# rpng/online_lang_splatting

Hardware: AMD Instinct MI355X
Metric: rasterizer fwd+bwd frames/sec @500k Gaussians, 1200x680, 15-dim lang (higher is better)
Workload: dtype f32

## Files before the change

include/olsr.h:

```cpp
#ifndef OLSR_H_INCLUDED
#define OLSR_H_INCLUDED

#include <stddef.h>
#include <stdint.h>

#ifdef __cplusplus
extern "C" {
#endif

#define OLSR_OK 0
#define OLSR_ERR_ARG (-1)
#define OLSR_ERR_DEVICE (-2)
#define OLSR_ERR_ALLOC (-3)
#define OLSR_ERR_CAPACITY (-4)

#define OLSR_STATUS_OK 0
#define OLSR_STATUS_OVERFLOW 1
#define OLSR_STATUS_SYNC_ERROR 2

#define OLSR_BWD_REFERENCE 0
#define OLSR_BWD_EXACT 1

typedef void *(*olsr_alloc_fn)(void *user, size_t nbytes);

// ... 277 lines not shown
  float obs_weight;
  float min_opacity;
  int32_t H, W;
  int32_t feat_layout;
  int32_t _pad0;
  const float *depth, *feat, *opacity;
} olsr_tsdf_view;
int olsr_tsdf_init(const olsr_tsdf_volume *volume, void *hip_stream);
int olsr_tsdf_integrate(const olsr_tsdf_volume *volume, int32_t n_views, const olsr_tsdf_view *views, void *hip_stream);
size_t olsr_tsdf_surface_scratch_bytes(int32_t X, int32_t Y, int32_t Z);
int olsr_tsdf_surface_plan(const olsr_tsdf_volume *volume, float min_weight, void *scratch, int32_t *status,
                           void *hip_stream);
int olsr_tsdf_surface_emit(const olsr_tsdf_volume *volume, float min_weight, const void *scratch, int32_t capacity,
                           float *points, float *feats, int32_t *voxel_index, void *hip_stream);

typedef struct olsr_pose_params {
  double lr_rot, lr_trans, lr_exposure;
  double beta1, beta2, eps;
  double converged_threshold;
  int32_t step;
  int32_t _pad0;
} olsr_pose_params;
int olsr_pose_step(const olsr_pose_params *params, const float *dL_dtau_sum, const float *dL_dexposure,
                   const float *projection_matrix, float *state, int32_t *status, void *hip_stream);
int olsr_pose_step_gated(const olsr_pose_params *params, const float *dL_dtau_sum, const float *dL_dexposure,
                         const float *projection_matrix, float *state, int32_t *status, const int32_t *frame_status,
                         void *hip_stream);

int olsr_accumulate_gradients(int32_t P, int32_t M, int32_t F, int32_t assign,
                              const float *dL_dmeans3D,
                              const float *dL_dsh, const float *dL_dopacity,
                              const float *dL_dscales, const float *dL_drotations,
                              const float *dL_dlanguage, const float *dL_dmeans2D,
                              const int32_t *radii, float *flat, float *densify,
                              int32_t *max_radii, void *hip_stream);

int olsr_sparse_exchange_mask(int32_t P, int32_t width, const float *flat, const uint64_t *row_mask,
                              const int32_t *max_radii, int32_t *imax, void *hip_stream);
int64_t olsr_sparse_exchange_scratch_ints(int32_t P);
int olsr_sparse_exchange_pack(int32_t P, int32_t width, int32_t capacity, const float *flat, const int32_t *imax,
                              int32_t *max_radii, uint64_t *row_mask, const float *densify, int32_t *idx,
                              float *fsum, int32_t *scratch, int32_t *status_dev, void *hip_stream);
int olsr_sparse_exchange_unpack(int32_t P, int32_t width, int32_t capacity, const int32_t *idx, const float *fsum,
                                float *flat, float *densify, void *hip_stream);

int olsr_mark_visible(int32_t P, const float *means3D, const float *viewmatrix,
                      const float *projmatrix, uint8_t *present, void *hip_stream);

const void *olsr_geometry_field(const void *geometry_buffer, int32_t P, int32_t F, const char *name);
const void *olsr_binning_field(const void *binning_buffer, int64_t num_rendered, int32_t F,
                               const char *name);
const void *olsr_image_field(const void *image_buffer, int32_t width, int32_t height, int32_t tile,
                             const char *name);

void olsr_set_profiling(int enable);
int olsr_get_stage_times(const char **names, float *ms, int max);

void olsr_debug_sort_timing(unsigned long long *device_buffer, int max_blocks, int max_launches);

int olsr_debug_sort_plan(int64_t n, int n_is_capacity, int32_t *keys_per_thread, int32_t *blocks);

void olsr_debug_sync_fault(int fault_bits, int spin_limit);

float olsr_debug_rows_ratio(int32_t packed_survivor_waves, float ratio, int32_t *redone_out);

void olsr_debug_sort_knobs(int keys_per_thread, int resident_blocks, int legacy);

void olsr_debug_sort_small(int enable);

void olsr_debug_sort_compact(int enable);

void olsr_debug_composite_stamps(unsigned long long *device_buffer, int capacity);

size_t olsr_debug_backward_ordered_scratch_bytes(int64_t num_rendered, int32_t F);
int olsr_debug_backward_ordered(const olsr_scene *scene, const void *geometry_buffer, int32_t num_rendered,
                                const void *binning_buffer, const void *image_buffer,
                                const float *dL_dout_color, const float *dL_dout_language, const float *dL_dout_depth,
                                void *scratch,
                                float *dL_dmeans2D, float *dL_dconic, float *dL_dopacity, float *dL_dcolors,
                                float *dL_dlanguage, float *dL_ddepths, int32_t condition, void *hip_stream);

int olsr_debug_sort_threads(int threads);

const char *olsr_last_error(void);
const char *olsr_version(void);

#ifdef __cplusplus
}
#endif
#endif
```

online_lang_splatting_amd/_abi.py:

```python
import ctypes as C

OLSR_OK = 0
OLSR_ERR_ARG = -1
OLSR_ERR_DEVICE = -2
OLSR_ERR_ALLOC = -3
OLSR_ERR_CAPACITY = -4

BWD_REFERENCE = 0
BWD_EXACT = 1

ACT_OPACITY_SIGMOID = 1
ACT_SCALE_EXP = 2
ACT_ROTATION_NORMALIZE = 4
ACT_ALL = 7
FLAG_SIGNED_EMPTY_RADII = 1
FLAG_FWD_ACCUM_WEIGHT = 4
FLAG_FRAMES_IN_FLIGHT = 8
FLAG_FWD_ACCUM_MFMA = 2

BINNING_RECT = 0
BINNING_ELLIPSE = 1

SUPPORTED_F = (0, 3, 15, 16, 32)
SUPPORTED_TILES = (15, 16)

ALLOC_FN = C.CFUNCTYPE(C.c_void_p, C.c_void_p, C.c_size_t)

_fp = C.c_void_p


class OlsrScene(C.Structure):

    _fields_ = [
        ("P", C.c_int32),
        ("D", C.c_int32),
        ("M", C.c_int32),
        ("F", C.c_int32),
        ("width", C.c_int32),
        ("height", C.c_int32),
        ("tile", C.c_int32),
        ("prefiltered", C.c_int32),
        ("debug", C.c_int32),
        ("bwd_mode", C.c_int32),
        ("tan_fovx", C.c_float),
        ("tan_fovy", C.c_float),
        ("scale_modifier", C.c_float),
        ("binning", C.c_int32),
        ("background", _fp),
        ("means3D", _fp),
        ("shs", _fp),
        ("colors_precomp", _fp),
        ("language_precomp", _fp),
        ("opacities", _fp),
        ("scales", _fp),
        ("rotations", _fp),
        ("cov3D_precomp", _fp),
        ("viewmatrix", _fp),
        ("projmatrix", _fp),
        ("projmatrix_raw", _fp),
        ("cam_pos", _fp),
        ("activations", C.c_int32),
        ("flags", C.c_int32),
        ("tile_depth_cut", _fp),
        ("backward_row_capacity", C.c_int64),
        ("depth_order_carry", _fp),
    ]


class OlsrGradBucket(C.Structure):

    _fields_ = [("flat", _fp), ("densify", _fp), ("max_radii", _fp), ("assign", C.c_int32), ("_pad0", C.c_int32),
                ("row_mask", _fp)]


class OlsrAdamParams(C.Structure):

    _fields_ = [(n, C.c_double) for n in ("lr_xyz", "lr_sh_dc", "lr_sh_rest", "lr_opacity", "lr_scale", "lr_rotation",
                                           "lr_language", "beta1", "beta2", "eps")] + [("step", C.c_int32), ("_pad0", C.c_int32)]


class OlsrAdamGroupParams(C.Structure):

    _fields_ = [("base", OlsrAdamParams), ("group_step", C.c_int32 * 7), ("skip_mask", C.c_int32)]


ADAM_GROUPS = ("xyz", "f_dc", "f_rest", "opacity", "scaling", "rotation", "f_language")

MAP_EDIT_DENSIFY, MAP_EDIT_MASK = 0, 1


class OlsrMapBuffers(C.Structure):

    _fields_ = [(n, _fp) for n in ("means3D", "shs", "opacities", "scales", "rotations", "language", "exp_avg", "exp_avg_sq",
                                   "kf_id", "n_obs", "stats", "max_radii")]


class OlsrMapEditParams(C.Structure):

    _fields_ = [("mode", C.c_int32), ("n_append", C.c_int32), ("append_kf_id", C.c_int32), ("screen_size_term", C.c_int32),
                ("max_grad", C.c_float), ("min_opacity", C.c_float), ("clone_max_scale", C.c_float), ("big_scale", C.c_float)]


class OlsrPoseParams(C.Structure):

# ... 100 lines not shown
```

online_lang_splatting_amd/_lib.py:

```python
import ctypes as C
import os

from . import _abi

_HERE = os.path.dirname(os.path.abspath(__file__))
LIB_PATH = os.environ.get("OLSR_LIB") or os.path.join(_HERE, "libolsr.so")

EXPORTS = (
    "olsr_geometry_bytes", "olsr_image_bytes", "olsr_binning_bytes", "olsr_backward_scratch_bytes", "olsr_last_forward_token", "olsr_live_rows", "olsr_forward", "olsr_forward_async", "olsr_forward_async_loss", "olsr_fused_loss_scratch_bytes",
    "olsr_backward", "olsr_accumulate_gradients", "olsr_sparse_exchange_mask", "olsr_sparse_exchange_scratch_ints", "olsr_sparse_exchange_pack", "olsr_sparse_exchange_unpack", "olsr_mapping_loss", "olsr_mapping_loss_scratch_bytes", "olsr_tracking_loss", "olsr_refinement_loss", "olsr_refinement_loss_scratch_bytes", "olsr_lang_ae_scratch_bytes", "olsr_lang_ae_train_step", "olsr_lang_ae_encode", "olsr_lang_ae_decode", "olsr_lang_query_scratch_bytes", "olsr_lang_query_sims", "olsr_lang_query_relevancy", "olsr_tsdf_init", "olsr_tsdf_integrate", "olsr_tsdf_surface_scratch_bytes", "olsr_tsdf_surface_plan", "olsr_tsdf_surface_emit", "olsr_pose_step", "olsr_pose_step_gated", "olsr_knn_mean_dist2", "olsr_knn_scratch_bytes", "olsr_adam_step", "olsr_adam_step_sum", "olsr_adam_step_masked", "olsr_adam_step_groups", "olsr_map_edit_scratch_bytes", "olsr_map_edit_plan", "olsr_map_edit_apply", "olsr_bucket_add", "olsr_mark_visible", "olsr_geometry_field", "olsr_binning_field", "olsr_image_field",
    "olsr_set_profiling", "olsr_get_stage_times", "olsr_debug_sort_timing", "olsr_debug_sort_plan", "olsr_debug_sort_knobs", "olsr_debug_sort_small", "olsr_debug_sort_compact", "olsr_debug_sort_threads", "olsr_debug_composite_stamps", "olsr_debug_sync_fault", "olsr_debug_rows_ratio", "olsr_debug_backward_ordered", "olsr_debug_backward_ordered_scratch_bytes", "olsr_live_rows_wait", "olsr_live_rows_overwritten", "olsr_backward_rows", "olsr_last_error", "olsr_version",
)

_lib = None


class OlsrError(RuntimeError):
    def __init__(self, code, msg):
        super().__init__(f"olsr error {code}: {msg}")
        self.code = code


def lib():
    global _lib
    if _lib is not None:
        return _lib
    if not os.path.exists(LIB_PATH):
        raise ImportError(
            f"{LIB_PATH} is missing: build it with `python -m online_lang_splatting_amd.build` "
            "(hipcc, gfx950).  There is no CPU or PyTorch fallback for the rasterizer.")
    L = C.CDLL(LIB_PATH)
    missing = [s for s in EXPORTS if not hasattr(L, s)]
    if missing:
        raise ImportError(f"{LIB_PATH} lacks symbols {missing}; rebuild it")
    vp, i32, i64, sz = C.c_void_p, C.c_int32, C.c_int64, C.c_size_t
    scene_p = C.POINTER(_abi.OlsrScene)
    L.olsr_geometry_bytes.argtypes, L.olsr_geometry_bytes.restype = [i32, i32], sz
    L.olsr_image_bytes.argtypes, L.olsr_image_bytes.restype = [i32, i32, i32], sz
    L.olsr_binning_bytes.argtypes, L.olsr_binning_bytes.restype = [i64, i32], sz
    L.olsr_forward.argtypes = [scene_p, _abi.ALLOC_FN, vp, _abi.ALLOC_FN, vp, _abi.ALLOC_FN, vp,
                               vp, vp, vp, vp, vp, vp, C.POINTER(i32), vp]
    L.olsr_forward.restype = C.c_int
    L.olsr_forward_async.argtypes = [scene_p, vp, vp, i64, vp, vp, vp, vp, vp, vp, vp, vp, vp, vp]
    L.olsr_forward_async.restype = C.c_int
    L.olsr_forward_async_loss.argtypes = [scene_p, vp, vp, i64, vp, vp, vp, vp, vp, vp, vp, vp, vp,
                                          C.POINTER(_abi.OlsrLossFusion), vp]
    L.olsr_forward_async_loss.restype = C.c_int
    L.olsr_fused_loss_scratch_bytes.argtypes, L.olsr_fused_loss_scratch_bytes.restype = [i32, i32, i32], sz
    L.olsr_backward_scratch_bytes.argtypes, L.olsr_backward_scratch_bytes.restype = [i64, i32], sz
    L.olsr_last_forward_token.argtypes, L.olsr_last_forward_token.restype = [], i32
    L.olsr_live_rows.argtypes, L.olsr_live_rows.restype = [i32, i32], i64
    L.olsr_live_rows_wait.argtypes, L.olsr_live_rows_wait.restype = [i32, i32, i32], i64
    L.olsr_live_rows_overwritten.argtypes, L.olsr_live_rows_overwritten.restype = [i32], i32
    L.olsr_backward_rows.argtypes, L.olsr_backward_rows.restype = [i32, i32, i64, i32], i64
    L.olsr_backward.argtypes = ([scene_p, vp, vp, i32, vp, vp, _abi.ALLOC_FN, vp, i32, vp, i64] + [vp] * 3 + [vp] * 13
                                + [C.POINTER(_abi.OlsrGradBucket), vp, vp])
    L.olsr_backward.restype = C.c_int
    L.olsr_accumulate_gradients.argtypes = [i32, i32, i32, i32] + [vp] * 12
    L.olsr_accumulate_gradients.restype = C.c_int
    L.olsr_sparse_exchange_mask.argtypes, L.olsr_sparse_exchange_mask.restype = [i32, i32] + [vp] * 5, C.c_int
    L.olsr_sparse_exchange_scratch_ints.argtypes, L.olsr_sparse_exchange_scratch_ints.restype = [i32], i64
    L.olsr_sparse_exchange_pack.argtypes, L.olsr_sparse_exchange_pack.restype = [i32, i32, i32] + [vp] * 10, C.c_int
    L.olsr_sparse_exchange_unpack.argtypes, L.olsr_sparse_exchange_unpack.restype = [i32, i32, i32] + [vp] * 5, C.c_int
    L.olsr_mapping_loss_scratch_bytes.argtypes, L.olsr_mapping_loss_scratch_bytes.restype = [i32, i32], sz
    L.olsr_mapping_loss.argtypes = [C.POINTER(_abi.OlsrLossParams)] + [vp] * 14
    L.olsr_mapping_loss.restype = C.c_int
    L.olsr_tracking_loss.argtypes = [C.POINTER(_abi.OlsrLossParams)] + [vp] * 13
    L.olsr_tracking_loss.restype = C.c_int
    L.olsr_refinement_loss_scratch_bytes.argtypes, L.olsr_refinement_loss_scratch_bytes.restype = [i32, i32], sz
    L.olsr_refinement_loss.argtypes, L.olsr_refinement_loss.restype = [i32, i32, C.c_float] + [vp] * 6, C.c_int
    L.olsr_lang_ae_scratch_bytes.argtypes, L.olsr_lang_ae_scratch_bytes.restype = [i32], sz
    L.olsr_lang_ae_train_step.argtypes = [C.POINTER(_abi.OlsrLangAeParams), i32] + [vp] * 10
    L.olsr_lang_ae_train_step.restype = C.c_int
    L.olsr_lang_ae_encode.argtypes, L.olsr_lang_ae_encode.restype = [i32, vp, vp, i32, vp, vp], C.c_int
    L.olsr_lang_ae_decode.argtypes, L.olsr_lang_ae_decode.restype = [i32, vp, vp, i32, vp, vp], C.c_int
    qp = C.POINTER(_abi.OlsrLangQueryParams)
    L.olsr_lang_query_scratch_bytes.argtypes, L.olsr_lang_query_scratch_bytes.restype = [qp], sz
    L.olsr_lang_query_sims.argtypes, L.olsr_lang_query_sims.restype = [qp] + [vp] * 6, C.c_int
    L.olsr_lang_query_relevancy.argtypes, L.olsr_lang_query_relevancy.restype = [qp] + [vp] * 11, C.c_int
    tv = C.POINTER(_abi.OlsrTsdfVolume)
    L.olsr_tsdf_init.argtypes, L.olsr_tsdf_init.restype = [tv, vp], C.c_int
    L.olsr_tsdf_integrate.argtypes, L.olsr_tsdf_integrate.restype = [tv, i32, C.POINTER(_abi.OlsrTsdfView), vp], C.c_int
    L.olsr_tsdf_surface_scratch_bytes.argtypes, L.olsr_tsdf_surface_scratch_bytes.restype = [i32, i32, i32], sz
    L.olsr_tsdf_surface_plan.argtypes, L.olsr_tsdf_surface_plan.restype = [tv, C.c_float, vp, vp, vp], C.c_int
    L.olsr_tsdf_surface_emit.argtypes, L.olsr_tsdf_surface_emit.restype = [tv, C.c_float, vp, i32, vp, vp, vp, vp], C.c_int
    L.olsr_pose_step.argtypes = [C.POINTER(_abi.OlsrPoseParams)] + [vp] * 6
    L.olsr_pose_step.restype = C.c_int
    L.olsr_pose_step_gated.argtypes = [C.POINTER(_abi.OlsrPoseParams)] + [vp] * 7
    L.olsr_pose_step_gated.restype = C.c_int
    L.olsr_adam_step.argtypes = [i32, i32, i32, C.POINTER(_abi.OlsrAdamParams)] + [vp] * 10
    L.olsr_adam_step.restype = C.c_int
    L.olsr_adam_step_sum.argtypes = [i32, i32, i32, C.POINTER(_abi.OlsrAdamParams), i32, C.POINTER(vp)] + [vp] * 9
    L.olsr_adam_step_sum.restype = C.c_int
    L.olsr_adam_step_masked.argtypes = [i32, i32, i32, C.POINTER(_abi.OlsrAdamParams), i32, C.POINTER(vp), C.POINTER(vp)] + [vp] * 9
    L.olsr_adam_step_masked.restype = C.c_int
    L.olsr_adam_step_groups.argtypes = [i32, i32, i32, C.POINTER(_abi.OlsrAdamGroupParams), i32, C.POINTER(vp), C.POINTER(vp)] + [vp] * 9
    L.olsr_adam_step_groups.restype = C.c_int
    L.olsr_map_edit_scratch_bytes.argtypes, L.olsr_map_edit_scratch_bytes.restype = [i32], sz
    mb, mp = C.POINTER(_abi.OlsrMapBuffers), C.POINTER(_abi.OlsrMapEditParams)
    L.olsr_map_edit_plan.argtypes, L.olsr_map_edit_plan.restype = [i32, mp, mb, vp, vp, vp, vp], C.c_int
    L.olsr_map_edit_apply.argtypes = [i32, i32, i32, mp, mb, vp, mb, vp, vp, i32, i32, mb, vp, vp]
    L.olsr_map_edit_apply.restype = C.c_int
    L.olsr_bucket_add.argtypes, L.olsr_bucket_add.restype = [i32, i32] + [vp] * 9, C.c_int
    L.olsr_knn_scratch_bytes.argtypes, L.olsr_knn_scratch_bytes.restype = [i32], sz
    L.olsr_knn_mean_dist2.argtypes, L.olsr_knn_mean_dist2.restype = [i32, vp, vp, vp, vp], C.c_int
    L.olsr_mark_visible.argtypes, L.olsr_mark_visible.restype = [i32, vp, vp, vp, vp, vp], C.c_int
    L.olsr_geometry_field.argtypes, L.olsr_geometry_field.restype = [vp, i32, i32, C.c_char_p], vp
    L.olsr_binning_field.argtypes, L.olsr_binning_field.restype = [vp, i64, i32, C.c_char_p], vp
    L.olsr_image_field.argtypes, L.olsr_image_field.restype = [vp, i32, i32, i32, C.c_char_p], vp
    L.olsr_set_profiling.argtypes, L.olsr_set_profiling.restype = [C.c_int], None
    L.olsr_get_stage_times.argtypes = [C.POINTER(C.c_char_p), C.POINTER(C.c_float), C.c_int]
    L.olsr_get_stage_times.restype = C.c_int
    L.olsr_debug_sort_plan.argtypes = [i64, C.c_int, C.POINTER(i32), C.POINTER(i32)]
    L.olsr_debug_sort_plan.restype = C.c_int
    L.olsr_debug_sort_knobs.argtypes = [C.c_int, C.c_int, C.c_int]
    L.olsr_debug_sort_knobs.restype = None
    L.olsr_debug_sort_small.argtypes, L.olsr_debug_sort_small.restype = [C.c_int], None
    L.olsr_debug_sort_compact.argtypes, L.olsr_debug_sort_compact.restype = [C.c_int], None
    L.olsr_debug_sort_threads.argtypes, L.olsr_debug_sort_threads.restype = [C.c_int], C.c_int
    L.olsr_debug_composite_stamps.argtypes, L.olsr_debug_composite_stamps.restype = [vp, C.c_int], None
    L.olsr_debug_sync_fault.argtypes = [C.c_int, C.c_int]
    L.olsr_debug_sync_fault.restype = None
    L.olsr_debug_rows_ratio.argtypes, L.olsr_debug_rows_ratio.restype = [i32, C.c_float, C.POINTER(i32)], C.c_float
    L.olsr_debug_backward_ordered_scratch_bytes.argtypes, L.olsr_debug_backward_ordered_scratch_bytes.restype = [i64, i32], sz
    L.olsr_debug_backward_ordered.argtypes = [scene_p, vp, i32, vp, vp] + [vp] * 3 + [vp] + [vp] * 6 + [i32, vp]
    L.olsr_debug_backward_ordered.restype = C.c_int
    L.olsr_last_error.argtypes, L.olsr_last_error.restype = [], C.c_char_p
    L.olsr_version.argtypes, L.olsr_version.restype = [], C.c_char_p
    _lib = L
    return L


def check(rc):
    if rc != 0:
        raise OlsrError(rc, lib().olsr_last_error().decode())


def stage_times(max_entries=1 << 16):
    names = (C.c_char_p * max_entries)()
    ms = (C.c_float * max_entries)()
    n = lib().olsr_get_stage_times(names, ms, max_entries)
    return [(names[i].decode(), float(ms[i])) for i in range(n)]


def set_profiling(enable):
    lib().olsr_set_profiling(1 if enable else 0)
```

online_lang_splatting_amd/csrc/k_order_carry.hip:

```cpp
#include <cstdlib>

#include "olsr_device.h"
#include "olsr_kernels.h"

namespace olsr {

constexpr int OC_W = 2048;
static_assert(OC_W == 2 * EMIT_CHUNK, "phase B leaves one instance total per emission block");

__device__ __forceinline__ int oc_count_less_front(const u64* __restrict__ B, int n, u64 x) {
  if (!(B[0] < x)) return 0;
  int lo = 0, step = 1;
  while (lo + step < n && B[lo + step] < x) {
    lo += step;
    step <<= 1;
  }
  int hi = lo + step < n ? lo + step : n;
  while (hi - lo > 1) {
    const int mid = (lo + hi) >> 1;
    if (B[mid] < x) lo = mid;
    else hi = mid;
  }
  return hi;
}
__device__ __forceinline__ int oc_count_leq_back(const u64* __restrict__ A, int n, u64 x) {
  if (A[n - 1] <= x) return n;
  int hi = n - 1, step = 1;
  while (hi - step >= 0 && A[hi - step] > x) {
    hi -= step;
    step <<= 1;
  }
  int lo = hi - step >= 0 ? hi - step : -1;
  while (hi - lo > 1) {
    const int mid = (lo + hi) >> 1;
    if (A[mid] <= x) lo = mid;
    else hi = mid;
  }
  return hi;
}

template <int T>
__device__ __forceinline__ u64* oc_window_sort(u64* a, u64* b) {
  constexpr int E = OC_W / T;
  const int tid = threadIdx.x;
#pragma unroll 1
  for (int run = 1; run < OC_W; run <<= 1) {
    u64 x[E];
    int dest[E];
#pragma unroll
    for (int k = 0; k < E; ++k) x[k] = a[tid + k * T];
#pragma unroll
    for (int k = 0; k < E; ++k) {
      const int i = tid + k * T;
      const int base = i & ~(2 * run - 1);
      if ((i & run) == 0) dest[k] = i + oc_count_less_front(a + base + run, run, x[k]);
      else dest[k] = i - run + oc_count_leq_back(a + base, run, x[k]);
    }
#pragma unroll
    for (int k = 0; k < E; ++k) b[dest[k]] = x[k];
    __syncthreads();
    u64* t = a;
    a = b;
    b = t;
  }
  return a;
}

__device__ __forceinline__ u64 oc_pad_low(int l) { return (u64)(u32)l; }
__device__ __forceinline__ u64 oc_pad_high(int l) { return 0xFFFFFFFF00000000ull | (u64)(u32)l; }

template <int T>
__global__ __launch_bounds__(T) void order_repair_a_kernel(int P, const u32* __restrict__ carry,
                                                           const u32* __restrict__ keys, u32* __restrict__ out_key,
                                                           u32* __restrict__ out_gid, u32* __restrict__ miss) {
  constexpr int E = OC_W / T;
  __shared__ __attribute__((aligned(16))) u64 s0[OC_W];
  __shared__ __attribute__((aligned(16))) u64 s1[OC_W];
  const int tid = threadIdx.x;
  const int base = (int)blockIdx.x * OC_W;
  bool bad = false;
#pragma unroll
  for (int k = 0; k < E; ++k) {
    const int l = tid + k * T, i = base + l;
    u64 c = oc_pad_high(l);
    if (i < P) {
      const u32 g = carry[i];
      const bool ok = g < (u32)P;
      bad |= !ok;
      c = ((u64)(ok ? keys[g] : 0xFFFFFFFFu) << 32) | (u64)g;
    }
    s0[l] = c;
  }
  __syncthreads();
  const u64* r = oc_window_sort<T>(s0, s1);
#pragma unroll
  for (int k = 0; k < E; ++k) {
    const int l = tid + k * T, i = base + l;
    if (i < P) {
      const u64 c = r[l];
      out_key[i] = (u32)(c >> 32);
      out_gid[i] = (u32)c;
    }
  }
  if (wave_any(bad) && lane_id() == 0) atomicOr(miss, 1u);
}

template <int T>
__global__ __launch_bounds__(T) void order_repair_b_kernel(int P, const u32* __restrict__ in_key,
                                                           const u32* __restrict__ in_gid, u32* __restrict__ carry,
                                                           const u32* __restrict__ inst_count, u64* __restrict__ totals,
                                                           u32* __restrict__ miss) {
  constexpr int E = OC_W / T;
  __shared__ __attribute__((aligned(16))) u64 s0[OC_W];
  __shared__ __attribute__((aligned(16))) u64 s1[OC_W];
  __shared__ u64 s_tot[2][T / 64];
  const int tid = threadIdx.x, lane = tid & 63, w = tid >> 6;
  const int start = (int)blockIdx.x * OC_W - OC_W / 2;
#pragma unroll
  for (int k = 0; k < E; ++k) {
    const int l = tid + k * T, i = start + l;
    u64 c;
    if (i < 0) c = oc_pad_low(l);
    else if (i < P) c = ((u64)in_key[i] << 32) | (u64)in_gid[i];
    else c = oc_pad_high(l);
    s0[l] = c;
  }
  __syncthreads();
  const u64* r = oc_window_sort<T>(s0, s1);
  bool bad = false;
// ... 68 lines not shown
```

online_lang_splatting_amd/csrc/olsr_device.h:

```cpp
#pragma once
#include <hip/hip_runtime.h>
#include <stdint.h>

#include "olsr_state.h"

namespace olsr {

__host__ __device__ __forceinline__ int32_t rows_stamp_of(long long row_capacity) {
  return row_capacity > 0 ? (int32_t)((row_capacity & 0x3FFFFFFFll) + 1) : 0;
}
__device__ __forceinline__ bool frame_unusable(const int32_t* counters, int32_t rows_stamp = 0) {
  return (counters[CNT_ROW_OVERFLOW] | counters[CNT_SYNC_ERROR]) != 0 ||
         (rows_stamp != 0 && counters[CNT_ROWS_STAMP] != rows_stamp);
}


typedef unsigned int u32;
typedef unsigned long long u64;

__device__ __forceinline__ int lane_id() { return (int)__builtin_amdgcn_mbcnt_hi(~0u, __builtin_amdgcn_mbcnt_lo(~0u, 0u)); }
__device__ __forceinline__ u64 ballot(bool p) { return __builtin_amdgcn_ballot_w64(p); }
__device__ __forceinline__ bool wave_any(bool p) { return ballot(p) != 0ull; }
__device__ __forceinline__ bool wave_all(bool p) { return ballot(!p) == 0ull; }

// ... 46 lines not shown
  float t = swap16_add(swap32_add(a, b), swap32_add(c, d));
  t += dpp_mov<0x128>(t);
  t += dpp_mov<0x124>(t);
  t += dpp_mov<0x122>(t);
  t += dpp_mov<0x121>(t);
  return t;
}
__device__ __forceinline__ float wave_reduce2(float a, float b) {
  float t = swap32_add(a, b);
  t += dpp_mov<0x128>(t);
  t += dpp_mov<0x124>(t);
  t += dpp_mov<0x122>(t);
  t += dpp_mov<0x121>(t);
  t += __builtin_bit_cast(float, __builtin_amdgcn_update_dpp(0, __builtin_bit_cast(int, t), 0x142, 0xa, 0xf, false));
  return t;
}
__device__ __forceinline__ void wave_lds_fence() {
  __builtin_amdgcn_fence(__ATOMIC_RELEASE, "wavefront");
  __builtin_amdgcn_wave_barrier();
}
__device__ __forceinline__ float wave_fold4_lds(float a, float b, float c, float d, float* wl) {
  const int l = lane_id();
  reinterpret_cast<float4*>(wl)[l] = make_float4(a, b, c, d);
  wave_lds_fence();
  const int r = l >> 4, col = l & 15;
  const float* p = wl + 4 * col + (((r & 1) << 1) | (r >> 1));
  const float t = (p[0] + p[64]) + (p[128] + p[192]);
  wave_lds_fence();
  return t;
}
__device__ __forceinline__ float wave_fold2_lds(float a, float b, float* wl) {
  const int l = lane_id();
  reinterpret_cast<float2*>(wl)[l] = make_float2(a, b);
  wave_lds_fence();
  const int r = l >> 4, col = l & 15;
  const float* p = wl + 2 * col + (r >> 1);
  const float t = (p[0] + p[32]) + (p[64] + p[96]);
  wave_lds_fence();
  return t;
}
template <int CTRL>
__device__ __forceinline__ float dpp_quad(float v) {
  return __builtin_bit_cast(float, __builtin_amdgcn_update_dpp(0, __builtin_bit_cast(int, v), CTRL, 0xf, 0xf, true));
}
__device__ __forceinline__ float row_sums3(float t0, float t1, float t2, bool in_hi8, bool in_0to3) {
  const float u0 = t0 + dpp_mov<0x128>(t0);
  const float u1 = t1 + dpp_mov<0x128>(t1);
  const float u2 = t2 + dpp_mov<0x128>(t2);
  float m = in_hi8 ? u1 : u0;
  m += dpp_mov<0x124>(m);
  const float v2 = u2 + dpp_mov<0x124>(u2);
  m = in_0to3 ? v2 : m;
  m += dpp_quad<0x4E>(m);
  m += dpp_quad<0xB1>(m);
  return m;
}
__device__ __forceinline__ float wave_reduce4_lds(float a, float b, float c, float d, float* wl) {
  float t = wave_fold4_lds(a, b, c, d, wl);
  t += dpp_mov<0x128>(t);
  t += dpp_mov<0x124>(t);
  t += dpp_mov<0x122>(t);
  t += dpp_mov<0x121>(t);
  return t;
}
__device__ __forceinline__ float wave_reduce2_lds(float a, float b, float* wl) {
  float t = wave_fold2_lds(a, b, wl);
  t += dpp_mov<0x128>(t);
  t += dpp_mov<0x124>(t);
  t += dpp_mov<0x122>(t);
  t += dpp_mov<0x121>(t);
  return t;
}
typedef float v2f __attribute__((ext_vector_type(2)));
__device__ __forceinline__ int reduce4_lane(int i) { return 16 * (((i & 1) << 1) | ((i >> 1) & 1)); }
__device__ __forceinline__ float lane_read(float v, int lane) {
  return __builtin_bit_cast(float, __builtin_amdgcn_readlane(__builtin_bit_cast(int, v), lane));
}

__device__ __forceinline__ float max_m87(float x) {
  float r;
  asm("v_max_f32 %0, 0xc2ae0000, %1" : "=v"(r) : "v"(x));
  return r;
}
__device__ __forceinline__ float pinned_expf(float x) {
  x = max_m87(x);
  float n = __builtin_rintf(x * 1.44269504088896341f);
  float r = __builtin_fmaf(n, -0.693359375f, x);
  r = __builtin_fmaf(n, 2.12194440e-4f, r);
  float p = 1.9875691500e-4f;
  p = __builtin_fmaf(p, r, 1.3981999507e-3f);
  p = __builtin_fmaf(p, r, 8.3334519073e-3f);
  p = __builtin_fmaf(p, r, 4.1665795894e-2f);
  p = __builtin_fmaf(p, r, 1.6666665459e-1f);
  p = __builtin_fmaf(p, r, 5.0000001201e-1f);
  float e = __builtin_fmaf(p, r * r, r) + 1.0f;
  int ni = (int)n;
  return e * bits2f((u32)(ni + 127) << 23);
}

typedef float v2f_ __attribute__((ext_vector_type(2)));
__device__ __forceinline__ v2f_ pinned_expf2(v2f_ x) {
  x.x = max_m87(x.x);
  x.y = max_m87(x.y);
  const v2f_ t = x * v2f_{1.44269504088896341f, 1.44269504088896341f};
  const v2f_ n = {__builtin_rintf(t.x), __builtin_rintf(t.y)};
  v2f_ r = __builtin_elementwise_fma(n, v2f_{-0.693359375f, -0.693359375f}, x);
  r = __builtin_elementwise_fma(n, v2f_{2.12194440e-4f, 2.12194440e-4f}, r);
  v2f_ p = {1.9875691500e-4f, 1.9875691500e-4f};
  p = __builtin_elementwise_fma(p, r, v2f_{1.3981999507e-3f, 1.3981999507e-3f});
  p = __builtin_elementwise_fma(p, r, v2f_{8.3334519073e-3f, 8.3334519073e-3f});
  p = __builtin_elementwise_fma(p, r, v2f_{4.1665795894e-2f, 4.1665795894e-2f});
  p = __builtin_elementwise_fma(p, r, v2f_{1.6666665459e-1f, 1.6666665459e-1f});
  p = __builtin_elementwise_fma(p, r, v2f_{5.0000001201e-1f, 5.0000001201e-1f});
  const v2f_ e = __builtin_elementwise_fma(p, r * r, r) + v2f_{1.0f, 1.0f};
  const v2f_ sc = {bits2f((u32)((int)n.x + 127) << 23), bits2f((u32)((int)n.y + 127) << 23)};
  return e * sc;
}

__device__ __forceinline__ int f2i_sat(float v) {
  if (v != v) return 0;
  if (v >= 2147483648.0f) return 2147483647;
  if (v <= -2147483648.0f) return (int)0x80000000;
  return (int)v;
}

__device__ __forceinline__ float fminf_ref(float a, float b) { return (b < a) ? b : a; }
__device__ __forceinline__ float fmaxf_ref(float a, float b) { return (a < b) ? b : a; }

__device__ __forceinline__ float ndc2Pix(float v, int S) { return (float)((((double)v + 1.0) * (double)S - 1.0) * 0.5); }

struct Rect { int x0, y0, x1, y1; };
template <int TILE>
__device__ __forceinline__ Rect get_rect(float px, float py, int max_radius, int gx, int gy) {
  Rect r;
  r.x0 = min(gx, max(0, f2i_sat((px - (float)max_radius) / (float)TILE)));
  r.y0 = min(gy, max(0, f2i_sat((py - (float)max_radius) / (float)TILE)));
  r.x1 = min(gx, max(0, f2i_sat((((px + (float)max_radius) + (float)TILE) - 1.0f) / (float)TILE)));
  r.y1 = min(gy, max(0, f2i_sat((((py + (float)max_radius) + (float)TILE) - 1.0f) / (float)TILE)));
  return r;
}

__device__ __forceinline__ float cull_threshold(float a, float b, float c, float opacity, int radius, int tile) {
  if (a != a || b != b || c != c || opacity != opacity) return 3e38f;
  const float o255 = 255.0f * opacity;
  if (!(o255 > 0.0f)) return -1.0f;
  const float L = __logf(o255);
  const float D = (float)radius + (float)tile + 1.0f;
  const float thr = L + 2e-3f + 1e-4f * fabsf(L) + 5e-7f * (fabsf(a) + fabsf(c) + fabsf(b)) * D * D;
  if (thr != thr) return 3e38f;
  if (!(thr >= 0.0f)) return -1.0f;
  return fminf(2.0f * thr * (1.0f + 1e-6f), 3e38f);
}

struct CullEllipse {
  float px, py, b, inv_a, A, det_lo, xstar, ystar, ymax;
  bool exact;
};
__device__ __forceinline__ CullEllipse cull_setup(float px, float py, float a, float b, float c, float t2, int radius) {
  CullEllipse e;
  e.px = px;
  e.py = py;
  e.b = b;
  const float w = b * b;
  const float err = __builtin_fmaf(-b, b, w);
  const float det = __builtin_fmaf(a, c, -w) + err;
  e.det_lo = det * (1.0f - 4e-7f);
  e.exact = (e.det_lo > 0.0f) && (a > 1e-30f) && (c > 1e-30f) && (t2 >= 0.0f) && (t2 < 1e6f) && (a < 1e6f) &&
            (c < 1e6f) && (radius < (1 << 20)) && (fabsf(px) < 1e7f) && (fabsf(py) < 1e7f);
  e.inv_a = e.exact ? __builtin_amdgcn_rcpf(a) : 0.0f;
  e.A = a * t2 * (1.0f + 4e-7f);
  const float inv_det = e.exact ? __builtin_amdgcn_rcpf(e.det_lo) * (1.0f + 4e-7f) : 0.0f;
  e.xstar = e.exact ? __builtin_amdgcn_sqrtf(t2 * c * inv_det) * (1.0f + 1e-6f) : 0.0f;
  e.ystar = e.exact ? -b * __builtin_amdgcn_rcpf(c) * e.xstar : 0.0f;
  e.ymax = e.exact ? __builtin_amdgcn_sqrtf(e.A * inv_det) * (1.0f + 1e-6f) : 3e38f;
  return e;
}
template <int TILE>
__device__ __forceinline__ void cull_rows(const CullEllipse& e, int ry0, int ry1, int& ya, int& yb) {
  ya = ry0;
  yb = ry1;
  if (!e.exact || !(e.ymax < 1e7f)) return;
  const float pad = 1e-2f + 4e-7f * (fabsf(e.py) + e.ymax);
  const float lo = floorf((e.py - e.ymax - pad) / (float)TILE), hi = floorf((e.py + e.ymax + pad) / (float)TILE);
  ya = max(ry0, (int)fmaxf(lo, -1.0f));
// ... 192 lines not shown
```

online_lang_splatting_amd/csrc/olsr_diag.hip:

```cpp
#include <hip/hip_runtime.h>

#include <cstdlib>
#include <cstring>
#include <vector>

#include "olsr_device.h"
#include "olsr_host.h"

using namespace olsr;

namespace {

thread_local bool g_profiling = false;
struct StageMark {
  const char* name;
  hipEvent_t ev;
};
thread_local std::vector<StageMark> g_marks;

void marks_reset() {
  for (auto& m : g_marks) (void)hipEventDestroy(m.ev);
  g_marks.clear();
}

struct StampState {
  unsigned long long* buf = nullptr;
  int capacity = 0;
  std::atomic<int> next{0};
} g_stamps;
__global__ void stamp_kernel(unsigned long long* slot, unsigned long long tag) {
  slot[0] = wall_clock64();
  slot[1] = tag;
}

}

namespace olsr {

void mark(const char* name, hipStream_t st) {
  if (!g_profiling || g_marks.size() >= (1u << 16)) return;
  StageMark m{name, nullptr};
  if (hipEventCreate(&m.ev) != hipSuccess) return;
  (void)hipEventRecord(m.ev, st);
  g_marks.push_back(m);
}

void stamp(hipStream_t st, int kind) {
  if (!g_stamps.buf) return;
  const int i = g_stamps.next.fetch_add(1);
  if (i >= g_stamps.capacity) return;
  stamp_kernel<<<1, 1, 0, st>>>(g_stamps.buf + 2 * (size_t)i, ((unsigned long long)(uintptr_t)st << 8) | (unsigned)kind);
}

SortKnobs& sort_knobs() {
  static SortKnobs k;
  return k;
}

}

namespace {
struct SortKnobsFromEnv {
  SortKnobsFromEnv() {
    auto num = [](const char* name) {
      const char* e = std::getenv(name);
      return e ? std::atoi(e) : 0;
    };
    sort_knobs().kpt = num("OLSR_SORT_KPT");
    sort_knobs().resident = num("OLSR_SORT_RESIDENT");
    sort_knobs().legacy = num("OLSR_SORT_LEGACY") == 1 ? 1 : 0;
    if (std::getenv("OLSR_SORT_SMALL")) sort_knobs().small_sort = num("OLSR_SORT_SMALL") != 0 ? 1 : 0;
    if (std::getenv("OLSR_SORT_COMPACT")) sort_knobs().compact = num("OLSR_SORT_COMPACT") != 0 ? 1 : 0;
    if (num("OLSR_SORT_THREADS") == 1024 || num("OLSR_SORT_THREADS") == 256) sort_knobs().threads = num("OLSR_SORT_THREADS");
  }
} g_sort_knobs_from_env;
}

extern "C" {

const void* olsr_geometry_field(const void* geometry_buffer, int32_t P, int32_t F, const char* name) {
  const GeometryState g = GeometryState::carve(const_cast<void*>(geometry_buffer), (size_t)P, grad_row(supported_F(F) ? F : 0));
  if (!std::strcmp(name, "depths")) return g.depths;
  if (!std::strcmp(name, "means2D")) return g.means2D;
  if (!std::strcmp(name, "cov3D")) return g.cov3D;
  if (!std::strcmp(name, "conic_opacity")) return g.conic_opacity;
  if (!std::strcmp(name, "rgb")) return g.rgb;
  if (!std::strcmp(name, "clamped")) return g.clamped;
  if (!std::strcmp(name, "tiles_touched")) return g.tiles_touched;
  if (!std::strcmp(name, "depth_order")) return g.depth_order;
  if (!std::strcmp(name, "depth_order_compacted")) return g.gacc;
  if (!std::strcmp(name, "counters")) return g.counters;
  if (!std::strcmp(name, "emit_totals")) return g.emit_status;
  if (!std::strcmp(name, "inst_start")) return g.inst_start;
  if (!std::strcmp(name, "blended")) return g.blended;
  if (!std::strcmp(name, "carry_miss")) return g.carry_miss;
  if (!std::strcmp(name, "carry_totals")) return g.carry_totals;
  if (!std::strcmp(name, "sort_keys")) return g.key_a;
  return nullptr;
}

const void* olsr_binning_field(const void* binning_buffer, int64_t num_rendered, int32_t F, const char* name) {
  (void)F;
  const BinningState b = BinningState::carve(const_cast<void*>(binning_buffer), (size_t)num_rendered);
  if (!std::strcmp(name, "inst_gid")) return b.inst_gid;
  if (!std::strcmp(name, "flags")) return b.flags;
  if (!std::strcmp(name, "rowbase")) return b.rowbase;
  if (!std::strcmp(name, "row_sync")) return b.tickets + BT_ROWS;
  if (!std::strcmp(name, "key_a")) return b.key_a;
  if (!std::strcmp(name, "key_b")) return b.key_b;
  if (!std::strcmp(name, "src")) return b.src;
  if (!std::strcmp(name, "val_b")) return b.val_b;
  return nullptr;
}

const void* olsr_image_field(const void* image_buffer, int32_t width, int32_t height, int32_t tile, const char* name) {
  const ImageState im =
      ImageState::carve(const_cast<void*>(image_buffer), (size_t)width * height, tile_count(width, height, tile));
  if (!std::strcmp(name, "final_T")) return im.final_T;
  if (!std::strcmp(name, "n_contrib")) return im.n_contrib;
  if (!std::strcmp(name, "ranges")) return im.ranges;
  if (!std::strcmp(name, "tile_work")) return im.tile_work;
  if (!std::strcmp(name, "tile_order")) return im.tile_order;
  return nullptr;
}

void olsr_set_profiling(int enable) {
  g_profiling = enable != 0;
  marks_reset();
}

int olsr_get_stage_times(const char** names, float* ms, int max) {
  if (g_marks.size() < 2) return 0;
  (void)hipEventSynchronize(g_marks.back().ev);
  int n = 0;
  for (size_t i = 1; i < g_marks.size() && n < max; ++i) {
    if (!std::strcmp(g_marks[i].name, "begin")) continue;
    float t = 0.f;
    if (hipEventElapsedTime(&t, g_marks[i - 1].ev, g_marks[i].ev) != hipSuccess) t = -1.f;
    names[n] = g_marks[i].name;
    ms[n] = t;
    ++n;
  }
  return n;
}

void olsr_debug_sort_timing(unsigned long long* device_buffer, int max_blocks, int max_launches) {
  debug_set_sort_timing(device_buffer, max_blocks, max_launches);
}

void olsr_debug_sync_fault(int fault_bits, int spin_limit) {
  if (fault_bits >= 0) sort_knobs().fault = fault_bits & 3;
  if (spin_limit >= 0) sort_knobs().spin_limit = spin_limit > 0 ? spin_limit : (1 << 22);
}

void olsr_debug_sort_knobs(int keys_per_thread, int resident_blocks, int legacy) {
  if (keys_per_thread >= 0) sort_knobs().kpt = keys_per_thread;
  if (resident_blocks >= 0) sort_knobs().resident = resident_blocks;
  if (legacy >= 0) sort_knobs().legacy = legacy ? 1 : 0;
}

void olsr_debug_composite_stamps(unsigned long long* device_buffer, int capacity) {
  g_stamps.buf = device_buffer;
  g_stamps.capacity = device_buffer ? capacity : 0;
  g_stamps.next = 0;
}

int olsr_debug_sort_threads(int threads) {
  if (threads == 0 || threads == 256 || threads == 1024) sort_knobs().threads = threads;
  return sort_knobs().threads.load();
}

void olsr_debug_sort_compact(int enable) {
  if (enable >= 0) sort_knobs().compact.store(enable ? 1 : 0, std::memory_order_relaxed);
}

void olsr_debug_sort_small(int enable) {
  if (enable >= 0) sort_knobs().small_sort = enable ? 1 : 0;
}

int olsr_debug_sort_plan(int64_t n, int n_is_capacity, int32_t* keys_per_thread, int32_t* blocks) {
  const SortPlan p = sort_plan((long long)n, n_is_capacity != 0);
  if (keys_per_thread) *keys_per_thread = p.kpt;
  if (blocks) *blocks = p.nblk;
  return fused_sort_applicable(n, 32) ? 1 : 0;
}

size_t olsr_debug_backward_ordered_scratch_bytes(int64_t num_rendered, int32_t F) {
  if (num_rendered < 0 || !supported_F(F)) return 0;
  return align_up((size_t)num_rendered * (size_t)grad_row(F) * sizeof(float)) + align_up((size_t)num_rendered) + 2 * ALIGN;
}

}
```

Baseline: 2401.

## Use magic-number rounding in pinned exp and early-exit sorted window passes

Rewrites pinned_expf and its paired form to get rint by adding and subtracting a magic constant, and to build the scale factor by shifting the float bits directly. This removes the rint and int-conversion instructions from the per-fragment exp, and the old versions are kept as reference functions. A new device sweep checks bit-exactness of the new exp against the reference over chosen input ranges. The order-carry window sort now checks whether the data is already ascending, globally and per merge pass, and skips work when it is; this adds block-wide reductions to every pass.

```diff
diff --git a/include/olsr.h b/include/olsr.h
--- a/include/olsr.h
+++ b/include/olsr.h
@@ -383,6 +383,8 @@
 
 int olsr_debug_sort_threads(int threads);
 
+int olsr_debug_exp_sweep(uint32_t first_bits, uint64_t count, uint64_t out[4]);
+
 const char *olsr_last_error(void);
 const char *olsr_version(void);
 
diff --git a/online_lang_splatting_amd/_abi.py b/online_lang_splatting_amd/_abi.py
--- a/online_lang_splatting_amd/_abi.py
+++ b/online_lang_splatting_amd/_abi.py
@@ -20,6 +20,9 @@
 
 BINNING_RECT = 0
 BINNING_ELLIPSE = 1
+
+EXP_SWEEP_RANGES = ((0x80000000, 0xC2B40000), (0x00000000, 0x42B00000))
+EXP_SWEEP_SPECIALS = (0x7F800000, 0xFF800000, 0x7FC00000, 0xFFC00000, 0xFFFFFFFF, 0xF149F2CA)
 
 SUPPORTED_F = (0, 3, 15, 16, 32)
 SUPPORTED_TILES = (15, 16)
diff --git a/online_lang_splatting_amd/_lib.py b/online_lang_splatting_amd/_lib.py
--- a/online_lang_splatting_amd/_lib.py
+++ b/online_lang_splatting_amd/_lib.py
@@ -9,7 +9,7 @@
 EXPORTS = (
     "olsr_geometry_bytes", "olsr_image_bytes", "olsr_binning_bytes", "olsr_backward_scratch_bytes", "olsr_last_forward_token", "olsr_live_rows", "olsr_forward", "olsr_forward_async", "olsr_forward_async_loss", "olsr_fused_loss_scratch_bytes",
     "olsr_backward", "olsr_accumulate_gradients", "olsr_sparse_exchange_mask", "olsr_sparse_exchange_scratch_ints", "olsr_sparse_exchange_pack", "olsr_sparse_exchange_unpack", "olsr_mapping_loss", "olsr_mapping_loss_scratch_bytes", "olsr_tracking_loss", "olsr_refinement_loss", "olsr_refinement_loss_scratch_bytes", "olsr_lang_ae_scratch_bytes", "olsr_lang_ae_train_step", "olsr_lang_ae_encode", "olsr_lang_ae_decode", "olsr_lang_query_scratch_bytes", "olsr_lang_query_sims", "olsr_lang_query_relevancy", "olsr_tsdf_init", "olsr_tsdf_integrate", "olsr_tsdf_surface_scratch_bytes", "olsr_tsdf_surface_plan", "olsr_tsdf_surface_emit", "olsr_pose_step", "olsr_pose_step_gated", "olsr_knn_mean_dist2", "olsr_knn_scratch_bytes", "olsr_adam_step", "olsr_adam_step_sum", "olsr_adam_step_masked", "olsr_adam_step_groups", "olsr_map_edit_scratch_bytes", "olsr_map_edit_plan", "olsr_map_edit_apply", "olsr_bucket_add", "olsr_mark_visible", "olsr_geometry_field", "olsr_binning_field", "olsr_image_field",
-    "olsr_set_profiling", "olsr_get_stage_times", "olsr_debug_sort_timing", "olsr_debug_sort_plan", "olsr_debug_sort_knobs", "olsr_debug_sort_small", "olsr_debug_sort_compact", "olsr_debug_sort_threads", "olsr_debug_composite_stamps", "olsr_debug_sync_fault", "olsr_debug_rows_ratio", "olsr_debug_backward_ordered", "olsr_debug_backward_ordered_scratch_bytes", "olsr_live_rows_wait", "olsr_live_rows_overwritten", "olsr_backward_rows", "olsr_last_error", "olsr_version",
+    "olsr_set_profiling", "olsr_get_stage_times", "olsr_debug_sort_timing", "olsr_debug_sort_plan", "olsr_debug_sort_knobs", "olsr_debug_sort_small", "olsr_debug_sort_compact", "olsr_debug_sort_threads", "olsr_debug_composite_stamps", "olsr_debug_sync_fault", "olsr_debug_rows_ratio", "olsr_debug_backward_ordered", "olsr_debug_backward_ordered_scratch_bytes", "olsr_debug_exp_sweep", "olsr_live_rows_wait", "olsr_live_rows_overwritten", "olsr_backward_rows", "olsr_last_error", "olsr_version",
 )
 
 _lib = None
@@ -125,6 +125,7 @@
     L.olsr_debug_backward_ordered_scratch_bytes.argtypes, L.olsr_debug_backward_ordered_scratch_bytes.restype = [i64, i32], sz
     L.olsr_debug_backward_ordered.argtypes = [scene_p, vp, i32, vp, vp] + [vp] * 3 + [vp] + [vp] * 6 + [i32, vp]
     L.olsr_debug_backward_ordered.restype = C.c_int
+    L.olsr_debug_exp_sweep.argtypes, L.olsr_debug_exp_sweep.restype = [C.c_uint32, C.c_uint64, C.POINTER(C.c_uint64)], C.c_int
     L.olsr_last_error.argtypes, L.olsr_last_error.restype = [], C.c_char_p
     L.olsr_version.argtypes, L.olsr_version.restype = [], C.c_char_p
     _lib = L
@@ -143,5 +144,11 @@
     return [(names[i].decode(), float(ms[i])) for i in range(n)]
 
 
+def exp_sweep(first_bits, count):
+    out = (C.c_uint64 * 4)()
+    check(lib().olsr_debug_exp_sweep(first_bits, count, out))
+    return int(out[0]), int(out[1]), int(out[2]), (None if out[3] == 2**64 - 1 else int(out[3]))
+
+
 def set_profiling(enable):
     lib().olsr_set_profiling(1 if enable else 0)
diff --git a/online_lang_splatting_amd/csrc/k_order_carry.hip b/online_lang_splatting_amd/csrc/k_order_carry.hip
--- a/online_lang_splatting_amd/csrc/k_order_carry.hip
+++ b/online_lang_splatting_amd/csrc/k_order_carry.hip
@@ -43,8 +43,18 @@
 __device__ __forceinline__ u64* oc_window_sort(u64* a, u64* b) {
   constexpr int E = OC_W / T;
   const int tid = threadIdx.x;
+  bool asc = true;
+#pragma unroll
+  for (int k = 0; k < E; ++k) {
+    const int i = tid + k * T;
+    if (i > 0) asc &= !(a[i] < a[i - 1]);
+  }
+  if (__syncthreads_and(asc)) return a;
 #pragma unroll 1
   for (int run = 1; run < OC_W; run <<= 1) {
+    bool in_order = true;
+    for (int h = run + tid * 2 * run; h < OC_W; h += T * 2 * run) in_order &= !(a[h] < a[h - 1]);
+    if (__syncthreads_and(in_order)) continue;
     u64 x[E];
     int dest[E];
 #pragma unroll
diff --git a/online_lang_splatting_amd/csrc/olsr_device.h b/online_lang_splatting_amd/csrc/olsr_device.h
--- a/online_lang_splatting_amd/csrc/olsr_device.h
+++ b/online_lang_splatting_amd/csrc/olsr_device.h
@@ -152,7 +152,46 @@
   asm("v_max_f32 %0, 0xc2ae0000, %1" : "=v"(r) : "v"(x));
   return r;
 }
+constexpr float EXP_MAGIC = 12582912.0f;
 __device__ __forceinline__ float pinned_expf(float x) {
+  x = max_m87(x);
+  const float tm = x * 1.44269504088896341f + EXP_MAGIC;
+  const float n = tm - EXP_MAGIC;
+  float r = __builtin_fmaf(n, -0.693359375f, x);
+  r = __builtin_fmaf(n, 2.12194440e-4f, r);
+  float p = 1.9875691500e-4f;
+  p = __builtin_fmaf(p, r, 1.3981999507e-3f);
+  p = __builtin_fmaf(p, r, 8.3334519073e-3f);
+  p = __builtin_fmaf(p, r, 4.1665795894e-2f);
+  p = __builtin_fmaf(p, r, 1.6666665459e-1f);
+  p = __builtin_fmaf(p, r, 5.0000001201e-1f);
+  const float q = __builtin_fmaf(p, r * r, r);
+  const float sc = bits2f((f2bits(tm) << 23) + 0x3F800000u);
+  return __builtin_fmaf(q, sc, sc);
+}
+
+typedef float v2f_ __attribute__((ext_vector_type(2)));
+typedef u32 v2u_ __attribute__((ext_vector_type(2)));
+__device__ __forceinline__ v2f_ pinned_expf2(v2f_ x) {
+  x.x = max_m87(x.x);
+  x.y = max_m87(x.y);
+  const v2f_ tm = x * v2f_{1.44269504088896341f, 1.44269504088896341f} + v2f_{EXP_MAGIC, EXP_MAGIC};
+  const v2f_ n = tm - v2f_{EXP_MAGIC, EXP_MAGIC};
+  v2f_ r = __builtin_elementwise_fma(n, v2f_{-0.693359375f, -0.693359375f}, x);
+  r = __builtin_elementwise_fma(n, v2f_{2.12194440e-4f, 2.12194440e-4f}, r);
+  v2f_ p = {1.9875691500e-4f, 1.9875691500e-4f};
+  p = __builtin_elementwise_fma(p, r, v2f_{1.3981999507e-3f, 1.3981999507e-3f});
+  p = __builtin_elementwise_fma(p, r, v2f_{8.3334519073e-3f, 8.3334519073e-3f});
+  p = __builtin_elementwise_fma(p, r, v2f_{4.1665795894e-2f, 4.1665795894e-2f});
+  p = __builtin_elementwise_fma(p, r, v2f_{1.6666665459e-1f, 1.6666665459e-1f});
+  p = __builtin_elementwise_fma(p, r, v2f_{5.0000001201e-1f, 5.0000001201e-1f});
+  const v2f_ q = __builtin_elementwise_fma(p, r * r, r);
+  const v2u_ sb = (__builtin_bit_cast(v2u_, tm) << 23) + v2u_{0x3F800000u, 0x3F800000u};
+  const v2f_ sc = __builtin_bit_cast(v2f_, sb);
+  return __builtin_elementwise_fma(q, sc, sc);
+}
+
+__device__ __forceinline__ float pinned_expf_ref(float x) {
   x = max_m87(x);
   float n = __builtin_rintf(x * 1.44269504088896341f);
   float r = __builtin_fmaf(n, -0.693359375f, x);
@@ -168,8 +207,7 @@
   return e * bits2f((u32)(ni + 127) << 23);
 }
 
-typedef float v2f_ __attribute__((ext_vector_type(2)));
-__device__ __forceinline__ v2f_ pinned_expf2(v2f_ x) {
+__device__ __forceinline__ v2f_ pinned_expf2_ref(v2f_ x) {
   x.x = max_m87(x.x);
   x.y = max_m87(x.y);
   const v2f_ t = x * v2f_{1.44269504088896341f, 1.44269504088896341f};
diff --git a/online_lang_splatting_amd/csrc/olsr_diag.hip b/online_lang_splatting_amd/csrc/olsr_diag.hip
--- a/online_lang_splatting_amd/csrc/olsr_diag.hip
+++ b/online_lang_splatting_amd/csrc/olsr_diag.hip
@@ -31,6 +31,33 @@
 __global__ void stamp_kernel(unsigned long long* slot, unsigned long long tag) {
   slot[0] = wall_clock64();
   slot[1] = tag;
+}
+
+__global__ __launch_bounds__(256) void exp_sweep_kernel(u32 first, unsigned long long count, unsigned long long* acc) {
+  const unsigned long long stride = (unsigned long long)gridDim.x * blockDim.x;
+  const unsigned long long shift = (count + 1) / 2;
+  unsigned long long bad_s = 0, bad_x = 0, bad_y = 0, first_bad = ~0ull;
+  for (unsigned long long i = (unsigned long long)blockIdx.x * blockDim.x + threadIdx.x; i < count; i += stride) {
+    const u32 pat = first + (u32)i;
+    unsigned long long j = i + shift;
+    if (j >= count) j -= count;
+    const u32 other = count > 1 ? first + (u32)j : (pat == 0xC1200000u ? 0xC1A00000u : 0xC1200000u);
+    const float a = bits2f(pat), b = bits2f(other);
+    const u32 ra = f2bits(pinned_expf_ref(a)), rb = f2bits(pinned_expf_ref(b));
+    const bool ms = f2bits(pinned_expf(a)) != ra;
+    const v2f_ nx = pinned_expf2(v2f_{a, b}), ox = pinned_expf2_ref(v2f_{a, b});
+    const bool mx = f2bits(nx.x) != f2bits(ox.x) || f2bits(nx.y) != f2bits(ox.y) || f2bits(nx.x) != ra || f2bits(nx.y) != rb;
+    const v2f_ ny = pinned_expf2(v2f_{b, a}), oy = pinned_expf2_ref(v2f_{b, a});
+    const bool my = f2bits(ny.x) != f2bits(oy.x) || f2bits(ny.y) != f2bits(oy.y) || f2bits(ny.x) != rb || f2bits(ny.y) != ra;
+    bad_s += ms;
+    bad_x += mx;
+    bad_y += my;
+    if ((ms || mx || my) && (unsigned long long)pat < first_bad) first_bad = pat;
+  }
+  if (bad_s) atomicAdd(acc + 0, bad_s);
+  if (bad_x) atomicAdd(acc + 1, bad_x);
+  if (bad_y) atomicAdd(acc + 2, bad_y);
+  if (first_bad != ~0ull) atomicMin(acc + 3, first_bad);
 }
 
 }
@@ -185,6 +212,24 @@
   return fused_sort_applicable(n, 32) ? 1 : 0;
 }
 
+int olsr_debug_exp_sweep(uint32_t first_bits, uint64_t count, uint64_t* out) {
+  if (out == nullptr || count > (1ull << 32) || (unsigned long long)first_bits + count > (1ull << 32)) return OLSR_ERR_ARG;
+  unsigned long long host[4] = {0ull, 0ull, 0ull, ~0ull};
+  unsigned long long* dev = nullptr;
+  if (hipMalloc(&dev, sizeof(host)) != hipSuccess) return OLSR_ERR_ALLOC;
+  bool ok = hipMemcpy(dev, host, sizeof(host), hipMemcpyHostToDevice) == hipSuccess;
+  if (ok && count > 0) {
+    const unsigned long long want = (count + 255) / 256;
+    exp_sweep_kernel<<<(unsigned)(want < 16384 ? want : 16384), 256>>>(first_bits, count, dev);
+    ok = hipGetLastError() == hipSuccess;
+  }
+  ok = ok && hipMemcpy(host, dev, sizeof(host), hipMemcpyDeviceToHost) == hipSuccess;
+  (void)hipFree(dev);
+  if (!ok) return OLSR_ERR_DEVICE;
+  for (int i = 0; i < 4; ++i) out[i] = host[i];
+  return OLSR_OK;
+}
+
 size_t olsr_debug_backward_ordered_scratch_bytes(int64_t num_rendered, int32_t F) {
   if (num_rendered < 0 || !supported_F(F)) return 0;
   return align_up((size_t)num_rendered * (size_t)grad_row(F) * sizeof(float)) + align_up((size_t)num_rendered) + 2 * ALIGN;
```

Result: faster. 2432, median of 6 (+1.3%).
